# LeeYN-43/Clover

Hardware: AMD Instinct MI355X
Metric: video-text pairs/sec (8f x 224^2, 32-tok), full pre-training step (higher is better)
Workload: dtype f16; 1 GPU; VideoSwin-T + BERT-base + 3-layer fusion, MLM + tri-modal exclusive InfoNCE + rank losses, 8f x 224^2, 32-tok; per_gpu_batch=8, global_batch=8, parallelism=dp1

## Files before the change

### clover_amd/_lib.py

```python
import ctypes as C
import os

_HERE = os.path.dirname(os.path.abspath(__file__))
HALF_F16 = os.environ.get('CLOVER_HALF', 'f16').lower() in ('f16', 'fp16', 'float16', 'half')
LIB_PATH = os.environ.get('CLOVER_LIB_PATH') or os.path.join(_HERE, 'libclover_hip_f16.so' if HALF_F16 else 'libclover_hip.so')


_scale_env = os.environ.get('CLOVER_LOSS_SCALE', '1024' if HALF_F16 else '1')
LOSS_SCALE_SPEC = 'dynamic' if _scale_env.strip().lower() == 'dynamic' else float(_scale_env)
LOSS_SCALE = (1024.0 if HALF_F16 else 1.0) if LOSS_SCALE_SPEC == 'dynamic' else LOSS_SCALE_SPEC


def half_dtype():
    import torch
    return torch.float16 if HALF_F16 else torch.bfloat16

ABI_VERSION = 18

ERRORS = {-1: 'CLV_ERR_ARG (bad argument)', -2: 'CLV_ERR_UNSUPPORTED (shape not supported by the kernels)',
          -3: 'CLV_ERR_LAUNCH (HIP launch failed)'}


class ClvAttnGeom(C.Structure):
    _fields_ = [(n, C.c_int32) for n in
# ... 82 lines not shown
    'clv_focal_ce_fwd': (C.c_int, [_p, _i32, _p, _p, _p, _p, _p, _i64, _i32, _f, _p]),
    'clv_focal_ce_bwd': (C.c_int, [_p, _i32, _p, _p, _p, _p, _p, _p, _i64, _i32, _f, _p]),
    'clv_focal_ce_fwd_ld': (C.c_int, [_p, _i32, _p, _p, _p, _p, _p, _i64, _i32, _i64, _f, _p]),
    'clv_focal_ce_bwd_ld': (C.c_int, [_p, _i32, _p, _p, _p, _p, _p, _p, _i64, _i32, _i64, _f, _p]),
    'clv_infonce_work_floats': (C.c_int64, [_i32, _i32]),
    'clv_infonce_fwd': (C.c_int, [_p] * 6 + [_i32, _i32, _i32, _f, _f, _p]),
    'clv_infonce_bwd': (C.c_int, [_p] * 10 + [_i32, _i32, _i32, _f, _f, _p]),
    'clv_infonce_pair_fwd': (C.c_int, [_p] * 4 + [_i32, _i32, _i32, _f, _f, _p]),
    'clv_infonce_pair_bwd': (C.c_int, [_p] * 4 + [_i32, _i32, _i32, _f, _f, _p]),
    'clv_normsoftmax_work_floats': (C.c_int64, [_i32, _i32]),
    'clv_normsoftmax_fwd': (C.c_int, [_p] * 5 + [_i32, _i32, _f, _f, _p]),
    'clv_normsoftmax_bwd': (C.c_int, [_p] * 6 + [_i32, _i32, _f, _p]),
    'clv_sumsq': (C.c_int, [_p, _p, _i64, _p]),
    'clv_adamw_step': (C.c_int, [_p] * 6 + [_i64] + [_f] * 9 + [_p]),
    'clv_gemm_nt_supported': (C.c_int, [_i64, _i32, _i32]),
    'clv_gemm_nt': (C.c_int, [_p] * 6 + [_i64, _i32, _i32, _i64, _i64, _i64, _i32, _p]),
    'clv_gemm_nt_work_bytes': (C.c_int64, [_i64, _i32, _i32]),
    'clv_gemm_nt_ex': (C.c_int, [_p] * 6 + [_i64, _i32, _i32, _i64, _i64, _i64, _i32, _p, _i64, _p]),
    'clv_transpose_batch': (C.c_int, [_p, _p, _p, _i32, _i32, _p]),
    'clv_layernorm_bwd_needs_reduce': (C.c_int, [_i64, _i32]),
    'clv_ln_reduce_batch': (C.c_int, [_p, _i32, _p]),
    'clv_linear_wgrad_in_place': (C.c_int, [C.c_int64, C.c_int32, C.c_int32]),
    'clv_linear_wgrad_class': (C.c_int, [C.c_int64, C.c_int32, C.c_int32]),
    'clv_linear_wgrad_batch_plan': (C.c_int, [_p, _i32]),
    'clv_linear_wgrad_batch': (C.c_int, [_p, _i32, _p]),
    'clv_linear_wgrad_batch_ss': (C.c_int, [_p, _i32, _p, _p]),
    'clv_linear_wgrad_splits': (C.c_int, [_i64, _i32, _i32]),
    'clv_wgrad_fold_batch': (C.c_int, [_p, _i32, _p]),
    'clv_wgrad_fold_batch_ss': (C.c_int, [_p, _i32, _p, _p]),
    'clv_optim_prep_slots': (C.c_int, [_p, _p, _p] + [_f] * 4 + [_p]),
    'clv_sumsq_ranges': (C.c_int, [_p, _p, _i32, _p, _p]),
    'clv_optim_prep': (C.c_int, [_p, _p] + [_f] * 4 + [_p]),
    'clv_adamw_step_dev': (C.c_int, [_p] * 6 + [_i64] + [_f] * 5 + [_p]),
    'clv_quant_fp8_rows': (C.c_int, [_p, _p, _p, _i64, _i32, _i64, _i64, _p]),
    'clv_gemm_nt_fp8_supported': (C.c_int, [_i64, _i32, _i32]),
    'clv_gemm_nt_fp8': (C.c_int, [_p] * 7 + [_i64, _i32, _i32, _i64, _i64, _i64, _i32, _p]),
    'clv_pack_bf16': (C.c_int, [_p, _p, _i64, _p]),
    'clv_sumsq_bf16': (C.c_int, [_p, _p, _i64, _p]),
    'clv_adamw_step_dev_bf16g': (C.c_int, [_p] * 6 + [_i64] + [_f] * 5 + [_p]),
    'clv_sgemm_strided': (C.c_int, [_p] * 4 + [_i64, _i32, _i32, _i64, _i64, _i64, _i64, _i64, _i32, _p]),
    'clv_sgemm_strided_rowsum': (C.c_int, [_p] * 4 + [_i64, _i32, _i32, _i64, _i64, _i64, _i64, _i64, _i32, _p]),
    'clv_sgemm_nt': (C.c_int, [_p] * 4 + [_i64, _i32, _i32, _i64, _i64, _i64, _p]),
    'clv_attn_f32_fwd': (C.c_int, [_p] * 7 + [C.POINTER(ClvAttnGeom), _i32, _p]),
    'clv_attn_f32_bwd_work_floats': (C.c_int64, [C.POINTER(ClvAttnGeom)]),
    'clv_attn_f32_bwd': (C.c_int, [_p] * 12 + [C.POINTER(ClvAttnGeom), _p]),
    'clv_qa_answer_rows': (C.c_int, [_p, _i32, _i32, _i32, _i32, _i32, _i64, _p, _p, _p]),
    'clv_qa_head_supported': (C.c_int, [_i32, _i32, _i32]),
    'clv_qa_head_fwd': (C.c_int, [_p] * 9 + [_f, _f] + [_p] * 5 + [_i32] * 4 + [_p]),
    'clv_qa_mc_ce_fwd': (C.c_int, [_p] * 4 + [_i32, _i32, _p]),
    'clv_qa_head_bwd': (C.c_int, [_p] * 14 + [_f] + [_p] * 9 + [_i32] * 4 + [_p]),
    'clv_attn_probs_mean': (C.c_int, [_p, _p, _p, _i32, _i32, _i32, _i32, _f, _p]),
    'clv_qa_choice_assemble': (C.c_int, [_p, _p, _p] + [_i32] * 5 + [_p]),
    'clv_qa_choice_assemble_bwd': (C.c_int, [_p, _p, _p] + [_i32] * 5 + [_p]),
}

_lib = None


def lib():
    global _lib
    if _lib is None:
        if not os.path.exists(LIB_PATH):
            raise RuntimeError(
                f'clover_amd: {LIB_PATH} is missing — the HIP extension is not built. '
                'Run `python __graft_entry__.py` (hipcc --offload-arch=gfx950). There is no CPU fallback.')
        L = C.CDLL(LIB_PATH)
        for name, (res, args) in SIGNATURES.items():
            fn = getattr(L, name)
            fn.restype = res
            fn.argtypes = args
        v = L.clv_abi_version()
        if v != ABI_VERSION:
            raise RuntimeError(f'clover_amd: ABI version mismatch (library {v}, binding {ABI_VERSION}); rebuild')
        if L.clv_half_type() != int(HALF_F16):
            raise RuntimeError(f'clover_amd: {LIB_PATH} computes in {"fp16" if L.clv_half_type() else "bf16"} but '
                               f'CLOVER_HALF asks for {"fp16" if HALF_F16 else "bf16"}')
        _lib = L
    return _lib


def check(rc, what):
    if rc != 0:
        raise RuntimeError(f'clover_amd: {what} failed: {ERRORS.get(rc, rc)}')
```

### clover_amd/backbones/cross_transformer.py

```python
import torch
import torch.nn as nn

from .. import ops
from ..builder import BACKBONES
from ..nn import LayerNorm, Linear, to_bf16, trunc_normal_
from .bert_layers import (BertEmbeddings, BertEncoder, extended_attention_mask, init_bert_weights,
                          load_pretrained_dir, resolve_bert_config)


@BACKBONES.register_module()
class CrossModalTransformerFromPretrained(nn.Module):
    def __init__(self, pretrained_model='bert-base-uncased', img_in_size=768, hidden_size=768, num_frames=4,
                 spacial_tokens=7 * 7, token_types=2, num_hidden_layers=12, layer_norm_eps=1e-12,
                 word_pos_start=False, use_prompt=False, use_text_cls=False, return_mask=False, bert_config=None,
                 **kwargs):
        super().__init__()
        cfg = resolve_bert_config(pretrained_model, bert_config, layer_norm_eps=layer_norm_eps,
                                  num_hidden_layers=num_hidden_layers)
        assert cfg['hidden_size'] == hidden_size, 'hidden_size must match the BERT config'
        self.bert_embedding = BertEmbeddings(cfg)
        self.bert_encoder = BertEncoder(cfg)
        init_bert_weights(self.bert_embedding)
        init_bert_weights(self.bert_encoder)
        load_pretrained_dir(self.bert_embedding, pretrained_model, prefix='bert.embeddings.')
        load_pretrained_dir(self.bert_encoder, pretrained_model, prefix='bert.encoder.',
                            allow_unexpected=tuple(f'layer.{i}.' for i in range(cfg['num_hidden_layers'], 64)))
        self.use_prompt = use_prompt
        if not use_text_cls:
            self.all_cls_token = nn.Parameter(torch.zeros(1, 1, hidden_size))
            trunc_normal_(self.all_cls_token, mean=0., std=.02)
            if self.use_prompt:
                self.prompt_token = nn.Parameter(torch.zeros(1, 4, hidden_size))
                trunc_normal_(self.prompt_token, mean=0., std=.02)
        else:
            self.all_cls_token = None
        self.vis_space_pos = nn.Parameter(0.02 * torch.randn(1, 1, spacial_tokens, hidden_size))
        self.vis_tempor_pos = nn.Parameter(0.02 * torch.randn(1, num_frames, 1, hidden_size))
        self.token_type_embeddings = nn.Embedding(token_types, hidden_size)
        self.norm = LayerNorm(hidden_size)
        self.word_pos_start = word_pos_start
        self.num_frames = num_frames
        self.spacial_tokens = spacial_tokens
        self.img_in_size = img_in_size
        self.hidden_size = hidden_size
        self.return_mask = return_mask
        if img_in_size != hidden_size:
            self.fc_in = Linear(img_in_size, hidden_size)
        self.fp16_enabled = False

    def _text_and_pos(self, text_embeddings, T, S, D):
        tt = self.token_type_embeddings.weight
        text = to_bf16(text_embeddings) + to_bf16(tt[1])
        pos = (self.vis_space_pos + self.vis_tempor_pos[:, :T, :, :]).reshape(1, T * S, D) + tt[0]
        return text, to_bf16(pos)

    def prepare(self, text_input_embeds, text_input_mask, B, T, S):
        D = self.hidden_size
        text = text_input_embeds
        mask = text_input_mask
        if text.shape[0] != B:
            text = text.view(B, -1, text.shape[-1])
            mask = mask.view(B, -1)
        text, pos = self._text_and_pos(text, T, S, D)
        n_vis = T * S + (1 if self.all_cls_token is not None else 0)
        mm_mask = torch.cat([torch.ones(B, n_vis, dtype=mask.dtype, device=text.device), mask], dim=1)
        return dict(key=(B, T, S), text=text, pos=pos, mask=mm_mask, ext_mask=extended_attention_mask(mm_mask))

    def forward(self, visual_token=None, text_input_ids=None, text_input_mask=None, text_input_embeds=None,
                num_choices=1, return_attention=False, **kwargs):
        if num_choices > 1:
            return self._forward_choices(visual_token, text_input_mask, text_input_embeds, num_choices, return_attention)
        if self.img_in_size != self.hidden_size:
            visual_token = self.fc_in(visual_token)
        B, T, S, D = visual_token.shape
        p_k_v_l = T * S + 1 if self.word_pos_start else 0
        if text_input_embeds is None:
            text_embeddings = self.bert_embedding(text_input_ids, past_key_values_length=p_k_v_l)
        else:
            text_embeddings = text_input_embeds
        if text_embeddings.shape[0] != B:
            text_embeddings = text_embeddings.view(B, -1, text_embeddings.shape[-1])
            text_input_mask = text_input_mask.view(B, -1)
        prepared = kwargs.get('prepared')
        if prepared is not None and prepared['key'] == (B, T, S) and not self.use_prompt:
            text_embeddings, pos, mm_mask_p, ext_mask_p = (prepared['text'], prepared['pos'], prepared['mask'],
                                                           prepared['ext_mask'])
        else:
            text_embeddings, pos = self._text_and_pos(text_embeddings, T, S, D)
            mm_mask_p = ext_mask_p = None
        visual = self.norm(to_bf16(visual_token.reshape(B, T * S, D)) + pos)
        if self.use_prompt:
            visual = torch.cat([visual, to_bf16(self.prompt_token).expand(B, -1, -1),
                                to_bf16(self.all_cls_token).expand(B, -1, -1)], dim=1)
            n_vis = T * S + 5
        elif self.all_cls_token is not None:
            visual = torch.cat([visual, to_bf16(self.all_cls_token).expand(B, -1, -1)], dim=1)
            n_vis = T * S + 1
        else:
            n_vis = T * S
        feat = torch.cat([visual, text_embeddings], dim=1)
        if mm_mask_p is not None:
            mm_mask, ext_mask = mm_mask_p, ext_mask_p
        else:
            mm_mask = torch.cat([torch.ones(B, n_vis, dtype=text_input_mask.dtype, device=feat.device),
                                 text_input_mask], dim=1)
            ext_mask = extended_attention_mask(mm_mask)
        h = self._encode(feat, ext_mask, return_attention)
        out = {'last_hidden_state': h,
               't_last_hidden_state': h[:, n_vis:],
               'v_last_hidden_state': h[:, :T * S]}
        if self.all_cls_token is not None:
            out['cls_last_hidden_state'] = h[:, n_vis - 1:n_vis]
        if return_attention:
            out['attention'] = self._last_attention
            self._last_attention = None
        if self.return_mask:
            return out, mm_mask
        return out

    def _encode(self, feat, ext_mask, return_attention):
        if not return_attention:
            return self.bert_encoder(feat, ext_mask)
        last = self.bert_encoder.layer[-1].attention.self
        last._clv_keep_qkv = True
        try:
            h = self.bert_encoder(feat, ext_mask)
            self._last_attention = ops.attn_probs_mean(last._clv_qkv, ext_mask, last.num_attention_heads)
        finally:
            last._clv_keep_qkv = False
            last._clv_qkv = None
        return h

    def _forward_choices(self, visual_token, text_input_mask, text_embeddings, C, return_attention):
        if self.use_prompt:
            raise NotImplementedError('num_choices > 1 with use_prompt=True: no Clover QA config uses prompt tokens')
        if self.img_in_size != self.hidden_size:
            visual_token = self.fc_in(visual_token)
        B, T, S, D = visual_token.shape
        BC = B * C
        text_embeddings = text_embeddings.view(BC, -1, text_embeddings.shape[-1])
        text_input_mask = text_input_mask.view(BC, -1)
        text_embeddings, pos = self._text_and_pos(text_embeddings, T, S, D)
        visual = self.norm(to_bf16(visual_token.reshape(B, T * S, D)) + pos)
        if self.all_cls_token is not None:
            visual = torch.cat([visual, to_bf16(self.all_cls_token).expand(B, -1, -1)], dim=1)
        n_vis = visual.shape[1]
        feat = _ChoiceAssemble.apply(visual, text_embeddings, C)
        mm_mask = torch.cat([torch.ones(BC, n_vis, dtype=text_input_mask.dtype, device=feat.device), text_input_mask],
                            dim=1)
        ext_mask = extended_attention_mask(mm_mask)
        h = self._encode(feat, ext_mask, return_attention)
        out = {'last_hidden_state': h, 't_last_hidden_state': h[:, n_vis:], 'v_last_hidden_state': h[:, :T * S]}
        if self.all_cls_token is not None:
            out['cls_last_hidden_state'] = h[:, n_vis - 1:n_vis]
        if return_attention:
            out['attention'] = self._last_attention
            self._last_attention = None
        if self.return_mask:
            return out, mm_mask
        return out


class _ChoiceAssemble(torch.autograd.Function):
# ... 11 lines not shown
```

### clover_amd/ops.py

```python
import ctypes as C

import os

import torch

from . import _lib, parity
from ._lib import ClvAttnGeom, check

BF16 = _lib.half_dtype()


def _stream():
    return C.c_void_p(torch.cuda.current_stream().cuda_stream)


def _ptr(t):
    return C.c_void_p(t.data_ptr()) if t is not None else C.c_void_p(0)


def _need_gpu(*ts):
    for t in ts:
        if t is not None and not t.is_cuda:
            raise RuntimeError('clover_amd ops run only on a HIP device (MI355X); there is no CPU fallback — '
                               'got a tensor on %s' % t.device)
# ... 1873 lines not shown
    def backward(ctx, dy):
        xb, *rest = ctx.saved_tensors
        weight, bias = ctx.refs
        Vp, V = ctx.Vp, weight.shape[0]
        R = xb.shape[0]
        base = getattr(dy, '_base', None)
        if (dy.dtype == BF16 and dy.stride() == (Vp, 1) and dy.storage_offset() == 0 and base is not None
                and tuple(base.shape) == (R, Vp) and getattr(base, '_clv_dscores_pad', 0) == Vp):
            dyp = base
            MLM_DECODER_STATS['in_place'] += 1
            if Vp > V:
                dyp[:, V:].zero_()
        else:
            MLM_DECODER_STATS['copied'] += 1
            dyp = torch.zeros(R, Vp, device=dy.device, dtype=BF16)
            dyp[:, :V].copy_(dy)
        if ctx.engine:
            dx = gemm_nt(dyp, weight._clv_pad_shadow_t) if ctx.needs_input_grad[0] else None
            linear_wgrad(dyp, xb, True, weight._clv_pad_grad, bias._clv_pad_grad)
            weight._clv_ready()
            bias._clv_ready()
            return dx, None, None
        Wp = rest[0]
        dx = gemm_nt(dyp, Wp.t().contiguous()) if ctx.needs_input_grad[0] else None
        global WGRAD_DEFER
        hold, WGRAD_DEFER = WGRAD_DEFER, None
        try:
            dwp, dbp = linear_wgrad(dyp, xb, True)
        finally:
            WGRAD_DEFER = hold
        return dx, dwp[:V].to(weight.dtype), dbp[:V].to(bias.dtype)


def mlm_decoder_ok(x, weight, bias):
    if parity.enabled() or not x.is_cuda or bias is None or os.environ.get('CLOVER_OWN_DECODER', '1') != '1':
        return False
    if all(hasattr(weight, a) for a in ('_clv_pad_shadow', '_clv_pad_shadow_t', '_clv_pad_grad')):
        return hasattr(bias, '_clv_pad_weight') and hasattr(bias, '_clv_pad_grad')
    return (not hasattr(weight, '_clv_pad_shadow') and weight.shape[1] % 64 == 0 and weight.shape[1] >= 64
            and x.shape[-1] == weight.shape[1])


def mlm_decoder(x, weight, bias):
    y = _MLMDecoder.apply(x.reshape(-1, x.shape[-1]), weight, bias)
    return y.view(x.shape[:-1] + (weight.shape[0],))


class _FusionTextOut(torch.autograd.Function):

    @staticmethod
    def forward(ctx, h, n_vis):
        B2, S, D = h.shape
        ctx.cfg = (B2, S, D, int(n_vis), h.dtype)
        t_last = h[:B2 // 2, n_vis:].contiguous()
        cls = h[:, n_vis].float().reshape(2, B2 // 2, D)
        return t_last, cls

    @staticmethod
    def backward(ctx, d_t, d_cls):
        B2, S, D, n_vis, dtype = ctx.cfg
        ref = d_t if d_t is not None else d_cls
        dh = torch.zeros(B2, S, D, device=ref.device, dtype=dtype)
        if d_t is not None:
            dh[:B2 // 2, n_vis:].copy_(d_t)
        if d_cls is not None:
            dh[:, n_vis].add_(d_cls.reshape(B2, D))
        return dh, None


def fusion_text_outputs(h, n_vis):
    assert h.dim() == 3 and h.shape[0] % 2 == 0 and 0 <= n_vis < h.shape[1]
    return _FusionTextOut.apply(h, int(n_vis))




class _FocalCE(torch.autograd.Function):
    @staticmethod
    def forward(ctx, logits, labels, gamma):
        _need_gpu(logits, labels)
        assert logits.dim() == 2 and logits.dtype in (BF16, torch.float32)
        strided = logits.stride(1) == 1 and logits.stride(0) > logits.shape[1] and logits.stride(0) % 2 == 0
        lg = logits if strided else _c(logits)
        lab = _c(labels.long())
        rows, V = lg.shape
        ld = lg.stride(0)
        dev = lg.device
        row_ce = torch.empty(rows, device=dev, dtype=torch.float32)
        row_lse = torch.empty_like(row_ce)
        acc = torch.zeros(2, device=dev, dtype=torch.float32)
        loss, count = acc[0:1], acc[1:2]
        check(_lib.lib().clv_focal_ce_fwd_ld(_ptr(lg), int(lg.dtype == BF16), _ptr(lab), _ptr(row_ce), _ptr(row_lse),
                                             _ptr(loss), _ptr(count), rows, V, ld, float(gamma), _stream()),
              'clv_focal_ce_fwd_ld')
        ctx.save_for_backward(lg, lab, row_ce, row_lse, count)
        ctx.gamma = float(gamma)
        return loss[0]

    @staticmethod
    def backward(ctx, dloss):
        lg, lab, row_ce, row_lse, count = ctx.saved_tensors
        rows, V = lg.shape
        ld = lg.stride(0)
        dl = _c(dloss.float().reshape(1))
        buf = torch.empty(rows, ld, device=lg.device, dtype=lg.dtype)
        if ld > V:
            buf._clv_dscores_pad = ld
        check(_lib.lib().clv_focal_ce_bwd_ld(_ptr(lg), int(lg.dtype == BF16), _ptr(lab), _ptr(row_ce), _ptr(row_lse),
                                             _ptr(count), _ptr(dl), _ptr(buf), rows, V, ld, ctx.gamma, _stream()),
              'clv_focal_ce_bwd_ld')
        return buf[:, :V], None, None


def focal_ce_masked(logits, labels, gamma=2.0):
    return _FocalCE.apply(logits, labels, gamma)


class _InfoNCE(torch.autograd.Function):
    @staticmethod
    def forward(ctx, e0, e1, e2, e3, temperature, margin):
        _need_gpu(e0)
        es = [_c(e.float()) for e in (e0, e1, e2, e3)]
        G, Dm = es[0].shape
        L = _lib.lib()
        work = torch.empty(L.clv_infonce_work_floats(G, Dm), device=e0.device, dtype=torch.float32)
# ... 362 lines not shown
```

### include/clover_hip.h

```cpp
#ifndef CLOVER_HIP_H
#define CLOVER_HIP_H
#include <stdint.h>

#ifdef __cplusplus
extern "C" {
#endif

#define CLV_ABI_VERSION 18
#define CLV_ERR_ARG (-1)
#define CLV_ERR_UNSUPPORTED (-2)
#define CLV_ERR_LAUNCH (-3)

int clv_abi_version(void);
int clv_half_type(void);

typedef struct ClvAttnGeom {
    int32_t mode;
    int32_t groups;
    int32_t N;
    int32_t nH;
    int32_t hd;
    int32_t D, H, W;
    int32_t wd, wh, ww;
    int32_t sd, sh, sw;
// ... 210 lines not shown
                       float lr, float beta1, float beta2, float eps, float weight_decay, void* stream);

int clv_sgemm_nt(const float* A, const float* B, const float* bias, float* C, int64_t M, int32_t N, int32_t K,
                 int64_t lda, int64_t ldb, int64_t ldc, void* stream);
int clv_sgemm_strided(const float* A, const float* B, const float* bias, float* C, int64_t M, int32_t N, int32_t K,
                      int64_t sai, int64_t sak, int64_t sbj, int64_t sbk, int64_t ldc, int32_t accumulate, void* stream);
int clv_sgemm_strided_rowsum(const float* A, const float* B, float* C, float* rowsum, int64_t M, int32_t N, int32_t K,
                             int64_t sai, int64_t sak, int64_t sbj, int64_t sbk, int64_t ldc, int32_t accumulate,
                             void* stream);
int clv_attn_f32_fwd(const float* q, const float* k, const float* v, float* o, const float* bias, const int32_t* rid,
                     const float* kmask, const ClvAttnGeom* geom, int32_t round_p, void* stream);
int64_t clv_attn_f32_bwd_work_floats(const ClvAttnGeom* geom);
int clv_attn_f32_bwd(const float* q, const float* k, const float* v, const float* dout, const float* bias,
                     const int32_t* rid, const float* kmask, float* dq, float* dk, float* dv, float* dbias, float* work,
                     const ClvAttnGeom* geom, void* stream);

int clv_patch_embed_fwd_fp8(const float* x, const void* w8, const float* wscale, const float* bias, const float* gamma,
                            const float* beta, const float* mask_token, const int64_t* vmask, void* out_clean,
                            void* out_masked, void* z_out, float* mean, float* rstd, int32_t B, int32_t T, int32_t H,
                            int32_t W, int32_t C, int32_t mh, int32_t mw, float eps, void* stream);
int clv_quant_fp8_rows(const void* x, void* q, float* scale, int64_t rows, int32_t K, int64_t ldx, int64_t ldq,
                       void* stream);
int clv_gemm_nt_fp8_supported(int64_t M, int32_t N, int32_t K);
int clv_gemm_nt_fp8(const void* a8, const void* b8, const float* sa, const float* sb, const float* bias, void* c, void* c2,
                    int64_t M, int32_t N, int32_t K, int64_t lda, int64_t ldb, int64_t ldc, int32_t epilogue,
                    void* stream);

int clv_pack_bf16(const float* src, void* dst, int64_t n, void* stream);
int clv_sumsq_bf16(const void* g, float* acc, int64_t n, void* stream);
int clv_adamw_step_dev_bf16g(float* p, const void* g, float* m, float* v, void* shadow, const void* state, int64_t n,
                             float lr, float beta1, float beta2, float eps, float weight_decay, void* stream);

int clv_qa_answer_rows(const int64_t* token_ids, int32_t N, int32_t L, int32_t Ltot, int32_t base, int32_t mode,
                       int64_t mask_id, int32_t* rows, int32_t* counts, void* stream);
int clv_qa_head_supported(int32_t D, int32_t H, int32_t K);
int clv_qa_head_fwd(const void* x, const int32_t* rows, const float* w1, const float* b1, const float* gamma,
                    const float* beta, const float* w2, const float* b2, const uint64_t* seed, float drop_p, float eps,
                    float* z, float* g, float* mean, float* rstd, float* logits, int32_t M, int32_t D, int32_t H, int32_t K,
                    void* stream);
int clv_qa_mc_ce_fwd(const float* logits, const int64_t* labels, float* dprob, float* out, int32_t B, int32_t C,
                     void* stream);
int clv_qa_head_bwd(const void* x, const int32_t* rows, const float* w1, const float* gamma, const float* beta,
                    const float* w2, const float* z, const float* g, const float* mean, const float* rstd, const float* dl,
                    const float* s1, const float* s2, const uint64_t* seed, float drop_p, float* dy, float* dz,
                    void* dx_full, float* dw1, float* db1, float* dgamma, float* dbeta, float* dw2, float* db2, int32_t M,
                    int32_t D, int32_t H, int32_t K, void* stream);
int clv_qa_choice_assemble(const void* visual, const void* text, void* feat, int32_t B, int32_t C, int32_t n_vis,
                           int32_t L, int32_t D, void* stream);
int clv_qa_choice_assemble_bwd(const void* dfeat, void* dvisual, void* dtext, int32_t B, int32_t C, int32_t n_vis,
                               int32_t L, int32_t D, void* stream);
int clv_attn_probs_mean(const void* qkv, const float* kmask, float* out, int32_t N, int32_t S, int32_t nH, int32_t hd,
                        float scale, void* stream);

#ifdef __cplusplus
}
#endif
#endif
```

Baseline: 768.5 pairs/s.

## Fuse cross-modal transformer input assembly and text-output slicing into HIP kernels

Adds HIP kernels that build the fusion-transformer input in one pass: visual+positional embedding add, LayerNorm, CLS/text concatenation with token-type embedding, and the extended attention mask. A matching backward kernel produces the visual and text grads and reduces the parameter grads through a two-stage partial-sum buffer. The text/CLS output slicing of the fusion output and its backward scatter also get dedicated kernels. The aim is to replace many small PyTorch elementwise, cat and reduction launches with a few kernels, at the cost of new custom code paths that bypass parity mode.

Result: no change. 767.9 pairs/s (median of 2 runs) (-0.1%).

```diff
diff --git a/clover_amd/_lib.py b/clover_amd/_lib.py
--- a/clover_amd/_lib.py
+++ b/clover_amd/_lib.py
@@ -158,6 +158,12 @@
     'clv_attn_probs_mean': (C.c_int, [_p, _p, _p, _i32, _i32, _i32, _i32, _f, _p]),
     'clv_qa_choice_assemble': (C.c_int, [_p, _p, _p] + [_i32] * 5 + [_p]),
     'clv_qa_choice_assemble_bwd': (C.c_int, [_p, _p, _p] + [_i32] * 5 + [_p]),
+    'clv_fusion_input_supported': (C.c_int, [_i32]),
+    'clv_fusion_input_fwd': (C.c_int, [_p] * 13 + [_i32] * 6 + [_f, _i32, _p]),
+    'clv_fusion_input_bwd_work_floats': (C.c_int64, [_i32] * 5),
+    'clv_fusion_input_bwd': (C.c_int, [_p] * 17 + [_i32] * 6 + [_p]),
+    'clv_fusion_text_out_fwd': (C.c_int, [_p] * 3 + [_i32] * 4 + [_p]),
+    'clv_fusion_text_out_bwd': (C.c_int, [_p] * 3 + [_i32] * 4 + [_p]),
 }
 
 _lib = None
diff --git a/clover_amd/backbones/cross_transformer.py b/clover_amd/backbones/cross_transformer.py
--- a/clover_amd/backbones/cross_transformer.py
+++ b/clover_amd/backbones/cross_transformer.py
@@ -54,6 +54,9 @@
         pos = (self.vis_space_pos + self.vis_tempor_pos[:, :T, :, :]).reshape(1, T * S, D) + tt[0]
         return text, to_bf16(pos)
 
+    def _glue_kernels(self, *ts):
+        return (not self.use_prompt and ops.glue_kernels_on(*ts) and self.vis_space_pos.is_cuda)
+
     def prepare(self, text_input_embeds, text_input_mask, B, T, S):
         D = self.hidden_size
         text = text_input_embeds
@@ -61,6 +64,10 @@
         if text.shape[0] != B:
             text = text.view(B, -1, text.shape[-1])
             mask = mask.view(B, -1)
+        if self._glue_kernels(text):
+            feat, ext_mask = ops.fusion_input_prepare(text, mask, T, S, self.token_type_embeddings.weight,
+                                                      self.all_cls_token)
+            return dict(key=(B, T, S), fused=True, feat=feat, ext_mask=ext_mask)
         text, pos = self._text_and_pos(text, T, S, D)
         n_vis = T * S + (1 if self.all_cls_token is not None else 0)
         mm_mask = torch.cat([torch.ones(B, n_vis, dtype=mask.dtype, device=text.device), mask], dim=1)
@@ -82,7 +89,23 @@
             text_embeddings = text_embeddings.view(B, -1, text_embeddings.shape[-1])
             text_input_mask = text_input_mask.view(B, -1)
         prepared = kwargs.get('prepared')
-        if prepared is not None and prepared['key'] == (B, T, S) and not self.use_prompt:
+        if prepared is not None and prepared['key'] != (B, T, S):
+            prepared = None
+        if self._glue_kernels(visual_token, text_embeddings):
+            ready = (prepared['feat'], prepared['ext_mask']) if prepared is not None and prepared.get('fused') else None
+            feat, ext_mask = ops.fusion_input(visual_token.reshape(B, T * S, D), text_embeddings, text_input_mask,
+                                              self.vis_space_pos, self.vis_tempor_pos, self.token_type_embeddings.weight,
+                                              self.all_cls_token, self.norm.weight, self.norm.bias, self.norm.eps, T, S,
+                                              prepared=ready)
+            n_vis = T * S + (1 if self.all_cls_token is not None else 0)
+            mm_mask = None
+            if self.return_mask:
+                mm_mask = torch.cat([torch.ones(B, n_vis, dtype=text_input_mask.dtype, device=feat.device),
+                                     text_input_mask], dim=1)
+            return self._outputs(feat, ext_mask, mm_mask, n_vis, T * S, return_attention)
+        if prepared is not None and prepared.get('fused'):
+            prepared = None
+        if prepared is not None and not self.use_prompt:
             text_embeddings, pos, mm_mask_p, ext_mask_p = (prepared['text'], prepared['pos'], prepared['mask'],
                                                            prepared['ext_mask'])
         else:
@@ -105,10 +128,13 @@
             mm_mask = torch.cat([torch.ones(B, n_vis, dtype=text_input_mask.dtype, device=feat.device),
                                  text_input_mask], dim=1)
             ext_mask = extended_attention_mask(mm_mask)
+        return self._outputs(feat, ext_mask, mm_mask, n_vis, T * S, return_attention)
+
+    def _outputs(self, feat, ext_mask, mm_mask, n_vis, TS, return_attention):
         h = self._encode(feat, ext_mask, return_attention)
         out = {'last_hidden_state': h,
                't_last_hidden_state': h[:, n_vis:],
-               'v_last_hidden_state': h[:, :T * S]}
+               'v_last_hidden_state': h[:, :TS]}
         if self.all_cls_token is not None:
             out['cls_last_hidden_state'] = h[:, n_vis - 1:n_vis]
         if return_attention:
diff --git a/clover_amd/csrc/glue.hip b/clover_amd/csrc/glue.hip
--- /dev/null
+++ b/clover_amd/csrc/glue.hip
@@ -0,0 +1,378 @@
+#include "common.hpp"
+#include "../../include/clover_hip.h"
+
+namespace {
+
+constexpr int GL_MAX_ITERS = 2;
+
+__device__ __forceinline__ float rnd16(float v) { return bf2f(f2bf(v)); }
+
+template <int ITERS>
+__device__ __forceinline__ void ld_half(const bf16_t* p, int C, int lane, float (&v)[ITERS][8]) {
+#pragma unroll
+    for (int i = 0; i < ITERS; ++i) {
+        const int c = (i * 64 + lane) * 8;
+        if (c < C) {
+            Frag8 f;
+            f.u4 = *reinterpret_cast<const uint4*>(p + c);
+#pragma unroll
+            for (int e = 0; e < 8; ++e) v[i][e] = bf2f(f.h[e]);
+        } else {
+#pragma unroll
+            for (int e = 0; e < 8; ++e) v[i][e] = 0.f;
+        }
+    }
+}
+
+template <int ITERS>
+__device__ __forceinline__ void st_half(bf16_t* p, int C, int lane, const float (&v)[ITERS][8]) {
+#pragma unroll
+    for (int i = 0; i < ITERS; ++i) {
+        const int c = (i * 64 + lane) * 8;
+        if (c < C) {
+            Frag8 f;
+#pragma unroll
+            for (int e = 0; e < 4; ++e) f.u[e] = pack2bf(v[i][2 * e], v[i][2 * e + 1]);
+            *reinterpret_cast<uint4*>(p + c) = f.u4;
+        }
+    }
+}
+
+template <int ITERS>
+__device__ __forceinline__ void ld_f32(const float* p, int C, int lane, float (&v)[ITERS][8]) {
+#pragma unroll
+    for (int i = 0; i < ITERS; ++i) {
+        const int c = (i * 64 + lane) * 8;
+        if (c < C) {
+            const float4 a = *reinterpret_cast<const float4*>(p + c), b = *reinterpret_cast<const float4*>(p + c + 4);
+            v[i][0] = a.x; v[i][1] = a.y; v[i][2] = a.z; v[i][3] = a.w;
+            v[i][4] = b.x; v[i][5] = b.y; v[i][6] = b.z; v[i][7] = b.w;
+        } else {
+#pragma unroll
+            for (int e = 0; e < 8; ++e) v[i][e] = 0.f;
+        }
+    }
+}
+
+template <int ITERS>
+__device__ __forceinline__ void pos_row(const float* sp, const float* tp, const float* tt, int t, int s, int C, int lane,
+                                        float (&pos)[ITERS][8]) {
+    float a[ITERS][8], b[ITERS][8], c0[ITERS][8];
+    ld_f32<ITERS>(sp + (int64_t)s * C, C, lane, a);
+    ld_f32<ITERS>(tp + (int64_t)t * C, C, lane, b);
+    ld_f32<ITERS>(tt, C, lane, c0);
+#pragma unroll
+    for (int i = 0; i < ITERS; ++i)
+#pragma unroll
+        for (int e = 0; e < 8; ++e) pos[i][e] = rnd16((a[i][e] + b[i][e]) + c0[i][e]);
+}
+
+template <int ITERS>
+__global__ void __launch_bounds__(256) fusion_input_fwd_kernel(
+    const bf16_t* __restrict__ visual, const bf16_t* __restrict__ text, const int64_t* __restrict__ mask,
+    const float* __restrict__ sp, const float* __restrict__ tp, const float* __restrict__ tt,
+    const float* __restrict__ cls, const float* __restrict__ gamma, const float* __restrict__ beta,
+    bf16_t* __restrict__ feat, float* __restrict__ ext, float* __restrict__ mean, float* __restrict__ rstd, int B2, int T,
+    int S, int L, int has_cls, int C, float eps, int parts) {
+    const int lane = threadIdx.x & 63;
+    const int TS = T * S, n_vis = TS + has_cls, St = n_vis + L;
+    const int rps = ((parts & 1) ? TS : 0) + ((parts & 2) ? St - TS : 0);
+    const int p0 = (parts & 1) ? 0 : TS;
+    const int64_t idx = (int64_t)blockIdx.x * 4 + (threadIdx.x >> 6);
+    if (idx >= (int64_t)B2 * rps) return;
+    const int b = (int)(idx / rps);
+    const int p = p0 + (int)(idx % rps);
+    bf16_t* out = feat + ((int64_t)b * St + p) * C;
+    if (p < TS) {
+        float x[ITERS][8], pos[ITERS][8];
+        pos_row<ITERS>(sp, tp, tt, p / S, p % S, C, lane, pos);
+        ld_half<ITERS>(visual + ((int64_t)b * TS + p) * C, C, lane, x);
+        float s = 0.f;
+#pragma unroll
+        for (int i = 0; i < ITERS; ++i) {
+            const bool live = (i * 64 + lane) * 8 < C;
+#pragma unroll
+            for (int e = 0; e < 8; ++e) {
+                x[i][e] = live ? rnd16(x[i][e] + pos[i][e]) : 0.f;
+                s += x[i][e];
+            }
+        }
+        const float invC = 1.0f / (float)C;
+        const float mu = wave_sum(s) * invC;
+        float vs = 0.f;
+#pragma unroll
+        for (int i = 0; i < ITERS; ++i)
+            if ((i * 64 + lane) * 8 < C) {
+#pragma unroll
+                for (int e = 0; e < 8; ++e) {
+                    const float d = x[i][e] - mu;
+                    vs += d * d;
+                }
+            }
+        const float rs = rsqrtf(wave_sum(vs) * invC + eps);
+        if (lane == 0) {
+            mean[(int64_t)b * TS + p] = mu;
+            rstd[(int64_t)b * TS + p] = rs;
+        }
+        float g[ITERS][8], bt[ITERS][8];
+        ld_f32<ITERS>(gamma, C, lane, g);
+        ld_f32<ITERS>(beta, C, lane, bt);
+#pragma unroll
+        for (int i = 0; i < ITERS; ++i)
+#pragma unroll
+            for (int e = 0; e < 8; ++e) x[i][e] = (x[i][e] - mu) * rs * g[i][e] + bt[i][e];
+        st_half<ITERS>(out, C, lane, x);
+        return;
+    }
+    float* em = ext + (int64_t)b * St;
+    if (p == TS)
+        for (int k = lane; k < TS; k += 64) em[k] = (1.0f - 1.0f) * -10000.0f;
+    float v[ITERS][8];
+    if (has_cls && p == TS) {
+        ld_f32<ITERS>(cls, C, lane, v);
+        if (lane == 0) em[p] = (1.0f - 1.0f) * -10000.0f;
+    } else {
+        const int l = p - n_vis;
+        float ty[ITERS][8];
+        ld_half<ITERS>(text + ((int64_t)b * L + l) * C, C, lane, v);
+        ld_f32<ITERS>(tt + C, C, lane, ty);
+#pragma unroll
+        for (int i = 0; i < ITERS; ++i)
+#pragma unroll
+            for (int e = 0; e < 8; ++e) v[i][e] += rnd16(ty[i][e]);
+        if (lane == 0) em[p] = (1.0f - (float)mask[(int64_t)b * L + l]) * -10000.0f;
+    }
+    st_half<ITERS>(out, C, lane, v);
+}
+
+template <int ITERS>
+__global__ void __launch_bounds__(256) fusion_input_bwd_kernel(
+    const bf16_t* __restrict__ dfeat, const bf16_t* __restrict__ visual, const float* __restrict__ sp,
+    const float* __restrict__ tp, const float* __restrict__ tt, const float* __restrict__ gamma,
+    const float* __restrict__ mean, const float* __restrict__ rstd, bf16_t* __restrict__ dvis,
+    bf16_t* __restrict__ dtext, float* __restrict__ part, int B2, int T, int S, int L, int has_cls, int C) {
+    constexpr int CW = ITERS * 512;
+    __shared__ float red[4][3][CW];
+    const int lane = threadIdx.x & 63, w = threadIdx.x >> 6;
+    const int TS = T * S, n_vis = TS + has_cls, St = n_vis + L;
+    const int p = blockIdx.x;
+    float a0[ITERS][8], a1[ITERS][8], a2[ITERS][8];
+#pragma unroll
+    for (int i = 0; i < ITERS; ++i)
+#pragma unroll
+        for (int e = 0; e < 8; ++e) a0[i][e] = a1[i][e] = a2[i][e] = 0.f;
+    if (p < TS) {
+        float pos[ITERS][8], gm[ITERS][8];
+        pos_row<ITERS>(sp, tp, tt, p / S, p % S, C, lane, pos);
+        ld_f32<ITERS>(gamma, C, lane, gm);
+        const float invC = 1.0f / (float)C;
+        for (int b = w; b < B2; b += 4) {
+            const int64_t row = (int64_t)b * TS + p;
+            float dy[ITERS][8], x[ITERS][8];
+            ld_half<ITERS>(dfeat + ((int64_t)b * St + p) * C, C, lane, dy);
+            ld_half<ITERS>(visual + row * C, C, lane, x);
+            const float mu = mean[row], rs = rstd[row];
+            float s1 = 0.f, s2 = 0.f;
+#pragma unroll
+            for (int i = 0; i < ITERS; ++i) {
+                const bool live = (i * 64 + lane) * 8 < C;
+#pragma unroll
+                for (int e = 0; e < 8; ++e) {
+                    const float xh = live ? (rnd16(x[i][e] + pos[i][e]) - mu) * rs : 0.f;
+                    x[i][e] = xh;
+                    a1[i][e] += dy[i][e] * xh;
+                    a2[i][e] += dy[i][e];
+                    dy[i][e] *= gm[i][e];
+                    s1 += dy[i][e];
+                    s2 += dy[i][e] * xh;
+                }
+            }
+            s1 = wave_sum(s1) * invC;
+            s2 = wave_sum(s2) * invC;
+#pragma unroll
+            for (int i = 0; i < ITERS; ++i)
+#pragma unroll
+                for (int e = 0; e < 8; ++e) {
+                    const float o = rnd16(rs * (dy[i][e] - s1 - x[i][e] * s2));
+                    dy[i][e] = o;
+                    a0[i][e] += o;
+                }
+            st_half<ITERS>(dvis + row * C, C, lane, dy);
+        }
+    } else {
+        for (int b = w; b < B2; b += 4) {
+            float d[ITERS][8];
+            ld_half<ITERS>(dfeat + ((int64_t)b * St + p) * C, C, lane, d);
+#pragma unroll
+            for (int i = 0; i < ITERS; ++i)
+#pragma unroll
+                for (int e = 0; e < 8; ++e) a0[i][e] += d[i][e];
+            if (p >= n_vis) st_half<ITERS>(dtext + ((int64_t)b * L + (p - n_vis)) * C, C, lane, d);
+        }
+    }
+#pragma unroll
+    for (int i = 0; i < ITERS; ++i)
+#pragma unroll
+        for (int e = 0; e < 8; ++e) {
+            const int c = (i * 64 + lane) * 8 + e;
+            red[w][0][c] = a0[i][e];
+            red[w][1][c] = a1[i][e];
+            red[w][2][c] = a2[i][e];
+        }
+    __syncthreads();
+    const int nk = p < TS ? 3 : 1;
+    for (int c = threadIdx.x; c < C; c += 256)
+        for (int k = 0; k < nk; ++k)
+            part[((int64_t)p * 3 + k) * C + c] = (red[0][k][c] + red[1][k][c]) + (red[2][k][c] + red[3][k][c]);
+}
+
+__global__ void __launch_bounds__(256) fusion_input_bwd_finish_kernel(const float* __restrict__ part, float* dsp, float* dtp,
+                                                                      float* dtt, float* dcls, float* dgamma, float* dbeta,
+                                                                      int T, int S, int L, int has_cls, int C) {
+    __shared__ float red[4][64];
+    const int lane = threadIdx.x & 63, w = threadIdx.x >> 6;
+    const int j = blockIdx.x, c = blockIdx.y * 64 + lane;
+    const int TS = T * S, n_vis = TS + has_cls;
+    int first = 0, step = 1, n = 0, k = 0;
+    float* dst = nullptr;
+    if (j < S) { first = j; step = S; n = T; dst = dsp + (int64_t)j * C; }
+    else if (j < S + T) { first = (j - S) * S; n = S; dst = dtp + (int64_t)(j - S) * C; }
+    else {
+        switch (j - S - T) {
+            case 0: n = TS; dst = dtt; break;
+            case 1: first = n_vis; n = L; dst = dtt + C; break;
+            case 2: first = TS; n = has_cls; dst = dcls; break;
+            case 3: n = TS; k = 1; dst = dgamma; break;
+            default: n = TS; k = 2; dst = dbeta; break;
+        }
+    }
+    float s = 0.f;
+    if (c < C)
+        for (int i = w; i < n; i += 4) s += part[((int64_t)(first + i * step) * 3 + k) * C + c];
+    red[w][lane] = s;
+    __syncthreads();
+    if (w == 0 && c < C && dst && n > 0) dst[c] += (red[0][lane] + red[1][lane]) + (red[2][lane] + red[3][lane]);
+}
+
+__global__ void __launch_bounds__(256) fusion_text_out_fwd_kernel(const bf16_t* __restrict__ h, bf16_t* __restrict__ t_last,
+                                                                  float* __restrict__ cls, int B2, int S, int D8, int n_vis) {
+    const int64_t e = (int64_t)blockIdx.x * 256 + threadIdx.x;
+    const int L = S - n_vis;
+    const int64_t nt = (int64_t)(B2 / 2) * L * D8, nc = (int64_t)B2 * D8;
+    if (e < nt) {
+        const int d = (int)(e % D8);
+        const int64_t row = e / D8;
+        const int l = (int)(row % L);
+        const int64_t b = row / L;
+        reinterpret_cast<uint4*>(t_last)[e] = reinterpret_cast<const uint4*>(h)[(b * S + n_vis + l) * D8 + d];
+    } else if (e < nt + nc) {
+        const int64_t f = e - nt;
+        const int d = (int)(f % D8);
+        const int64_t b = f / D8;
+        Frag8 v;
+        v.u4 = reinterpret_cast<const uint4*>(h)[(b * S + n_vis) * D8 + d];
+        float4* o = reinterpret_cast<float4*>(cls + f * 8);
+        o[0] = make_float4(bf2f(v.h[0]), bf2f(v.h[1]), bf2f(v.h[2]), bf2f(v.h[3]));
+        o[1] = make_float4(bf2f(v.h[4]), bf2f(v.h[5]), bf2f(v.h[6]), bf2f(v.h[7]));
+    }
+}
+
+__global__ void __launch_bounds__(256) fusion_text_out_bwd_kernel(const bf16_t* __restrict__ d_t, const float* __restrict__ d_cls,
+                                                                  bf16_t* __restrict__ dh, int B2, int S, int D8, int n_vis) {
+    const int64_t e = (int64_t)blockIdx.x * 256 + threadIdx.x;
+    if (e >= (int64_t)B2 * S * D8) return;
+    const int d = (int)(e % D8);
+    const int64_t row = e / D8;
+    const int r = (int)(row % S);
+    const int64_t b = row / S;
+    const int L = S - n_vis;
+    Frag8 v;
+    v.u4 = make_uint4(0, 0, 0, 0);
+    if (d_t && r >= n_vis && b < B2 / 2) v.u4 = reinterpret_cast<const uint4*>(d_t)[(b * L + (r - n_vis)) * D8 + d];
+    if (d_cls && r == n_vis) {
+        const float4* c = reinterpret_cast<const float4*>(d_cls + (b * D8 + d) * 8);
+        const float4 c0 = c[0], c1 = c[1];
+        v.u[0] = pack2bf(bf2f(v.h[0]) + c0.x, bf2f(v.h[1]) + c0.y);
+        v.u[1] = pack2bf(bf2f(v.h[2]) + c0.z, bf2f(v.h[3]) + c0.w);
+        v.u[2] = pack2bf(bf2f(v.h[4]) + c1.x, bf2f(v.h[5]) + c1.y);
+        v.u[3] = pack2bf(bf2f(v.h[6]) + c1.z, bf2f(v.h[7]) + c1.w);
+    }
+    reinterpret_cast<uint4*>(dh)[e] = v.u4;
+}
+
+bool geom_ok(int B2, int T, int S, int L, int has_cls, int C) {
+    return B2 > 0 && T > 0 && S > 0 && L > 0 && (has_cls == 0 || has_cls == 1) && C > 0 &&
+           (int64_t)B2 * ((int64_t)T * S + 1 + L) < (1ll << 30);
+}
+
+}
+
+extern "C" int clv_fusion_input_supported(int32_t C) { return C > 0 && C % 8 == 0 && C <= 64 * 8 * GL_MAX_ITERS; }
+
+extern "C" int clv_fusion_input_fwd(const void* visual, const void* text, const int64_t* mask, const float* space_pos,
+                                    const float* tempor_pos, const float* type_emb, const float* cls, const float* gamma,
+                                    const float* beta, void* feat, float* ext_mask, float* mean, float* rstd, int32_t B2,
+                                    int32_t T, int32_t S, int32_t L, int32_t has_cls, int32_t C, float eps, int32_t parts,
+                                    void* stream) {
+    if (!feat || !geom_ok(B2, T, S, L, has_cls, C) || parts < 1 || parts > 3) return CLV_ERR_ARG;
+    if ((parts & 1) && (!visual || !space_pos || !tempor_pos || !type_emb || !gamma || !beta || !mean || !rstd))
+        return CLV_ERR_ARG;
+    if ((parts & 2) && (!text || !mask || !type_emb || !ext_mask || (has_cls && !cls))) return CLV_ERR_ARG;
+    if (!clv_fusion_input_supported(C)) return CLV_ERR_UNSUPPORTED;
+    const int TS = T * S;
+    const int64_t rows = (int64_t)B2 * (((parts & 1) ? TS : 0) + ((parts & 2) ? has_cls + L : 0));
+    const dim3 grid((unsigned)((rows + 3) / 4));
+    hipStream_t st = (hipStream_t)stream;
+#define CLV_FI_ARGS (const bf16_t*)visual, (const bf16_t*)text, mask, space_pos, tempor_pos, type_emb, cls, gamma, beta, \
+                    (bf16_t*)feat, ext_mask, mean, rstd, B2, T, S, L, has_cls, C, eps, parts
+    if (C <= 512) hipLaunchKernelGGL(fusion_input_fwd_kernel<1>, grid, dim3(256), 0, st, CLV_FI_ARGS);
+    else hipLaunchKernelGGL(fusion_input_fwd_kernel<2>, grid, dim3(256), 0, st, CLV_FI_ARGS);
+#undef CLV_FI_ARGS
+    return clv_check_launch();
+}
+
+extern "C" int64_t clv_fusion_input_bwd_work_floats(int32_t T, int32_t S, int32_t L, int32_t has_cls, int32_t C) {
+    return ((int64_t)T * S + has_cls + L) * 3 * C;
+}
+
+extern "C" int clv_fusion_input_bwd(const void* dfeat, const void* visual, const float* space_pos, const float* tempor_pos,
+                                    const float* type_emb, const float* gamma, const float* mean, const float* rstd,
+                                    void* dvisual, void* dtext, float* work, float* dspace_pos, float* dtempor_pos,
+                                    float* dtype_emb, float* dcls, float* dgamma, float* dbeta, int32_t B2, int32_t T,
+                                    int32_t S, int32_t L, int32_t has_cls, int32_t C, void* stream) {
+    if (!dfeat || !visual || !space_pos || !tempor_pos || !type_emb || !gamma || !mean || !rstd || !dvisual || !dtext ||
+        !work || !dspace_pos || !dtempor_pos || !dtype_emb || !dgamma || !dbeta || (has_cls && !dcls) ||
+        !geom_ok(B2, T, S, L, has_cls, C))
+        return CLV_ERR_ARG;
+    if (!clv_fusion_input_supported(C)) return CLV_ERR_UNSUPPORTED;
+    const int St = T * S + has_cls + L;
+    hipStream_t st = (hipStream_t)stream;
+#define CLV_FI_ARGS (const bf16_t*)dfeat, (const bf16_t*)visual, space_pos, tempor_pos, type_emb, gamma, mean, rstd, \
+                    (bf16_t*)dvisual, (bf16_t*)dtext, work, B2, T, S, L, has_cls, C
+    if (C <= 512) hipLaunchKernelGGL(fusion_input_bwd_kernel<1>, dim3(St), dim3(256), 0, st, CLV_FI_ARGS);
+    else hipLaunchKernelGGL(fusion_input_bwd_kernel<2>, dim3(St), dim3(256), 0, st, CLV_FI_ARGS);
+#undef CLV_FI_ARGS
+    hipLaunchKernelGGL(fusion_input_bwd_finish_kernel, dim3(S + T + 5, (C + 63) / 64), dim3(256), 0, st, work, dspace_pos,
+                       dtempor_pos, dtype_emb, dcls, dgamma, dbeta, T, S, L, has_cls, C);
+    return clv_check_launch();
+}
+
+extern "C" int clv_fusion_text_out_fwd(const void* h, void* t_last, float* cls, int32_t B2, int32_t S, int32_t D,
+                                       int32_t n_vis, void* stream) {
+    if (!h || !t_last || !cls || B2 <= 0 || (B2 & 1) || S <= 0 || D <= 0 || n_vis < 0 || n_vis >= S) return CLV_ERR_ARG;
+    if (D % 8) return CLV_ERR_UNSUPPORTED;
+    const int64_t total = ((int64_t)(B2 / 2) * (S - n_vis) + B2) * (D / 8);
+    hipLaunchKernelGGL(fusion_text_out_fwd_kernel, dim3((unsigned)((total + 255) / 256)), dim3(256), 0, (hipStream_t)stream,
+                       (const bf16_t*)h, (bf16_t*)t_last, cls, B2, S, D / 8, n_vis);
+    return clv_check_launch();
+}
+
+extern "C" int clv_fusion_text_out_bwd(const void* d_t, const float* d_cls, void* dh, int32_t B2, int32_t S, int32_t D,
+                                       int32_t n_vis, void* stream) {
+    if (!dh || B2 <= 0 || (B2 & 1) || S <= 0 || D <= 0 || n_vis < 0 || n_vis >= S) return CLV_ERR_ARG;
+    if (D % 8) return CLV_ERR_UNSUPPORTED;
+    const int64_t total = (int64_t)B2 * S * (D / 8);
+    hipLaunchKernelGGL(fusion_text_out_bwd_kernel, dim3((unsigned)((total + 255) / 256)), dim3(256), 0, (hipStream_t)stream,
+                       (const bf16_t*)d_t, d_cls, (bf16_t*)dh, B2, S, D / 8, n_vis);
+    return clv_check_launch();
+}
diff --git a/clover_amd/ops.py b/clover_amd/ops.py
--- a/clover_amd/ops.py
+++ b/clover_amd/ops.py
@@ -1949,6 +1949,16 @@
     def forward(ctx, h, n_vis):
         B2, S, D = h.shape
         ctx.cfg = (B2, S, D, int(n_vis), h.dtype)
+        ctx.fused = glue_kernels_on(h)
+        if ctx.fused:
+            if h.dtype != BF16:
+                raise TypeError(f'fusion_text_outputs takes {BF16} rows on the device, got {h.dtype}')
+            h = _c(h)
+            t_last = torch.empty(B2 // 2, S - n_vis, D, device=h.device, dtype=h.dtype)
+            cls = torch.empty(2, B2 // 2, D, device=h.device, dtype=torch.float32)
+            check(_lib.lib().clv_fusion_text_out_fwd(_ptr(h), _ptr(t_last), _ptr(cls), B2, S, D, int(n_vis), _stream()),
+                  'clv_fusion_text_out_fwd')
+            return t_last, cls
         t_last = h[:B2 // 2, n_vis:].contiguous()
         cls = h[:, n_vis].float().reshape(2, B2 // 2, D)
         return t_last, cls
@@ -1957,6 +1967,13 @@
     def backward(ctx, d_t, d_cls):
         B2, S, D, n_vis, dtype = ctx.cfg
         ref = d_t if d_t is not None else d_cls
+        if ctx.fused:
+            dt = _c(d_t if d_t.dtype == dtype else d_t.to(dtype)) if d_t is not None else None
+            dc = _c(d_cls.float()) if d_cls is not None else None
+            dh = torch.empty(B2, S, D, device=ref.device, dtype=dtype)
+            check(_lib.lib().clv_fusion_text_out_bwd(_ptr(dt), _ptr(dc), _ptr(dh), B2, S, D, n_vis, _stream()),
+                  'clv_fusion_text_out_bwd')
+            return dh, None
         dh = torch.zeros(B2, S, D, device=ref.device, dtype=dtype)
         if d_t is not None:
             dh[:B2 // 2, n_vis:].copy_(d_t)
@@ -1968,6 +1985,138 @@
 def fusion_text_outputs(h, n_vis):
     assert h.dim() == 3 and h.shape[0] % 2 == 0 and 0 <= n_vis < h.shape[1]
     return _FusionTextOut.apply(h, int(n_vis))
+
+
+def glue_kernels_on(*ts):
+    return not parity.enabled() and all(t.is_cuda for t in ts if t is not None)
+
+
+def _fi_rows(t, what):
+    if t.dtype != BF16:
+        t = t.to(BF16)
+    t = _c(t)
+    assert t.data_ptr() % 16 == 0, f'fusion_input: {what} rows are not 16-byte aligned'
+    return t
+
+
+def _fi_param(p, shape_tail, what):
+    if p.dtype != torch.float32 or not p.is_contiguous() or tuple(p.shape[-len(shape_tail):]) != tuple(shape_tail):
+        raise TypeError(f'fusion_input: {what} must be a contiguous fp32 tensor ending in {tuple(shape_tail)}, got '
+                        f'{p.dtype} {tuple(p.shape)}')
+    return p
+
+
+def fusion_input_prepare(text, mask, T, S, type_emb, cls):
+    with torch.no_grad():
+        text = _fi_rows(text.detach(), 'text')
+        B2, L, D = text.shape
+        has_cls = int(cls is not None)
+        St = T * S + has_cls + L
+        m = _c(mask.detach().reshape(B2, L))
+        if m.dtype != torch.int64:
+            m = m.long()
+        tt = _fi_param(type_emb.detach(), (D,), 'type_emb')
+        c = _fi_param(cls.detach(), (D,), 'cls') if has_cls else None
+        feat = torch.empty(B2, St, D, device=text.device, dtype=BF16)
+        ext = torch.empty(B2, St, device=text.device, dtype=torch.float32)
+        check(_lib.lib().clv_fusion_input_fwd(None, _ptr(text), _ptr(m), None, None, _ptr(tt), _ptr(c), None, None,
+                                              _ptr(feat), _ptr(ext), None, None, B2, int(T), int(S), L, has_cls, D, 0.0,
+                                              2, _stream()), 'clv_fusion_input_fwd')
+    return feat, ext
+
+
+class _FusionInput(torch.autograd.Function):
+
+    @staticmethod
+    def forward(ctx, visual, text, mask, sp, tp, tt, cls, gamma, beta, eps, T, S, prepared):
+        _need_gpu(visual, text, mask)
+        L_ = _lib.lib()
+        visual = _fi_rows(visual, 'visual')
+        B2, TS, D = visual.shape
+        assert TS == T * S and text.shape[0] == B2 and text.shape[2] == D, (visual.shape, text.shape, T, S)
+        if not L_.clv_fusion_input_supported(D):
+            raise RuntimeError(f'CLV_ERR_UNSUPPORTED: fusion_input width {D} (a multiple of 8 up to 1024)')
+        L = text.shape[1]
+        has_cls = int(cls is not None)
+        St = TS + has_cls + L
+        _fi_param(sp, (S, D), 'vis_space_pos')
+        _fi_param(tp, (1, D), 'vis_tempor_pos')
+        assert tp.numel() >= T * D and tt.shape[0] >= 2, 'fusion_input: more frames than temporal positions / < 2 token types'
+        _fi_param(tt, (D,), 'type_emb')
+        _fi_param(gamma, (D,), 'gamma')
+        _fi_param(beta, (D,), 'beta')
+        if has_cls:
+            _fi_param(cls, (D,), 'cls')
+        mean = torch.empty(B2 * TS, device=visual.device, dtype=torch.float32)
+        rstd = torch.empty_like(mean)
+        if prepared is None:
+            text_r = _fi_rows(text, 'text')
+            m = _c(mask.reshape(B2, L))
+            if m.dtype != torch.int64:
+                m = m.long()
+            feat = torch.empty(B2, St, D, device=visual.device, dtype=BF16)
+            ext = torch.empty(B2, St, device=visual.device, dtype=torch.float32)
+            parts = 3
+        else:
+            feat, ext = prepared
+            assert tuple(feat.shape) == (B2, St, D) and feat.dtype == BF16 and feat.is_contiguous(), feat.shape
+            text_r = m = None
+            parts = 1
+        check(L_.clv_fusion_input_fwd(_ptr(visual), _ptr(text_r), _ptr(m), _ptr(sp), _ptr(tp), _ptr(tt), _ptr(cls),
+                                      _ptr(gamma), _ptr(beta), _ptr(feat), _ptr(ext), _ptr(mean), _ptr(rstd), B2, int(T),
+                                      int(S), L, has_cls, D, float(eps), parts, _stream()), 'clv_fusion_input_fwd')
+        ctx.save_for_backward(visual, sp, tp, tt, gamma, mean, rstd)
+        ctx.params = (sp, tp, tt, cls, gamma, beta)
+        ctx.geom = (B2, int(T), int(S), L, has_cls, D)
+        ctx.text_dtype = text.dtype
+        ctx.mark_non_differentiable(ext)
+        return feat, ext
+
+    @staticmethod
+    def backward(ctx, dfeat, _dext):
+        visual, sp, tp, tt, gamma, mean, rstd = ctx.saved_tensors
+        B2, T, S, L, has_cls, D = ctx.geom
+        L_ = _lib.lib()
+        d = _fi_rows(dfeat, 'd feat')
+        dvis = torch.empty_like(visual)
+        dtext = torch.empty(B2, L, D, device=d.device, dtype=BF16)
+        work = torch.empty(L_.clv_fusion_input_bwd_work_floats(T, S, L, has_cls, D), device=d.device, dtype=torch.float32)
+        dests, loose = [], []
+        for p in ctx.params:
+            sink = getattr(p, '_clv_grad', None) if p is not None else None
+            if sink is not None and sink.dtype == torch.float32 and sink.is_contiguous():
+                dests.append(sink)
+            else:
+                dests.append(None)
+                if p is not None:
+                    loose.append(p.numel())
+        if loose:
+            buf = torch.zeros(sum((n + 7) // 8 * 8 for n in loose), device=d.device, dtype=torch.float32)
+            off = 0
+            for i, p in enumerate(ctx.params):
+                if p is not None and dests[i] is None:
+                    dests[i] = buf[off:off + p.numel()].view(p.shape)
+                    off += (p.numel() + 7) // 8 * 8
+        check(L_.clv_fusion_input_bwd(_ptr(d), _ptr(visual), _ptr(sp), _ptr(tp), _ptr(tt), _ptr(gamma), _ptr(mean),
+                                      _ptr(rstd), _ptr(dvis), _ptr(dtext), _ptr(work), *[_ptr(t) for t in dests], B2, T, S,
+                                      L, has_cls, D, _stream()), 'clv_fusion_input_bwd')
+        grads = []
+        for i, p in enumerate(ctx.params):
+            if p is None:
+                grads.append(None)
+            elif dests[i] is getattr(p, '_clv_grad', None):
+                p._clv_ready()
+                grads.append(None)
+            else:
+                grads.append(dests[i].to(p.dtype) if ctx.needs_input_grad[3 + i] else None)
+        if dtext.dtype != ctx.text_dtype:
+            dtext = dtext.to(ctx.text_dtype)
+        return (dvis, dtext, None, *grads, None, None, None, None)
+
+
+def fusion_input(visual, text, mask, space_pos, tempor_pos, type_emb, cls, gamma, beta, eps, T, S, prepared=None):
+    return _FusionInput.apply(visual, text, mask, space_pos, tempor_pos, type_emb, cls, gamma, beta, float(eps), int(T),
+                              int(S), prepared)
 
 
 
diff --git a/include/clover_hip.h b/include/clover_hip.h
--- a/include/clover_hip.h
+++ b/include/clover_hip.h
@@ -286,6 +286,22 @@
 int clv_attn_probs_mean(const void* qkv, const float* kmask, float* out, int32_t N, int32_t S, int32_t nH, int32_t hd,
                         float scale, void* stream);
 
+int clv_fusion_input_supported(int32_t C);
+int clv_fusion_input_fwd(const void* visual, const void* text, const int64_t* mask, const float* space_pos,
+                         const float* tempor_pos, const float* type_emb, const float* cls, const float* gamma,
+                         const float* beta, void* feat, float* ext_mask, float* mean, float* rstd, int32_t B2, int32_t T,
+                         int32_t S, int32_t L, int32_t has_cls, int32_t C, float eps, int32_t parts, void* stream);
+int64_t clv_fusion_input_bwd_work_floats(int32_t T, int32_t S, int32_t L, int32_t has_cls, int32_t C);
+int clv_fusion_input_bwd(const void* dfeat, const void* visual, const float* space_pos, const float* tempor_pos,
+                         const float* type_emb, const float* gamma, const float* mean, const float* rstd, void* dvisual,
+                         void* dtext, float* work, float* dspace_pos, float* dtempor_pos, float* dtype_emb, float* dcls,
+                         float* dgamma, float* dbeta, int32_t B2, int32_t T, int32_t S, int32_t L, int32_t has_cls,
+                         int32_t C, void* stream);
+int clv_fusion_text_out_fwd(const void* h, void* t_last, float* cls, int32_t B2, int32_t S, int32_t D, int32_t n_vis,
+                            void* stream);
+int clv_fusion_text_out_bwd(const void* d_t, const float* d_cls, void* dh, int32_t B2, int32_t S, int32_t D, int32_t n_vis,
+                            void* stream);
+
 #ifdef __cplusplus
 }
 #endif
```
